# sashashura/h2o-3

Hardware: AMD Instinct MI355X
Metric: gbm_trees_per_sec (higher is better)
Workload: dtype fp32; 1 GPU; model=GBM binomial 100Mx100 ntrees=500 max_depth=8, rows=100000000, cols=100, max_depth=8, histogram_type=QuantilesGlobal, nbins=255, global_batch=100000000, parallelism=dp1

## Files before the change

### h2o3_amd/models/tree/devtree.py

```python
from __future__ import annotations

import ctypes
import os

import numpy as np
import torch

from ...ops import tree_ops
from ...ops.tree_ops import _ptr, _stream
from ...parallel import cloud
from ...parallel import collectives as coll
from ...utils import graphs
from .engine import _TreeBuf

RS = 16
(GAIN, FEAT, T, OPT, L0, L1, R0, R1, T0, T1, OK, NL, NAW, ST, CT, VAL) = range(16)
MAX_DEPTH = 11
_cv, _ci, _cll, _cd, _cf = ctypes.c_void_p, ctypes.c_int, ctypes.c_longlong, ctypes.c_double, ctypes.c_float


def _libs():
    from ...ops import _native
    lh = tree_ops._lib()
    ls = _native.get_lib("tree_split")
    if not getattr(lh, "_typed_dt", False):
        lh.h2o_dt_items.argtypes = [_ci, _cv, _ci, _ci, _ci, _ci, _ci, _cv, _cv, _cv, _cv]
        lh.h2o_dt_offsets.argtypes = [_cv, _cv, _cv, _cv, _ci, _cv, _cv, _cv, _cv]
        lh.h2o_dt_sibling.argtypes = [_cv, _cv, _cv, _ci, _ci, _ci, _ci, _ci, _ci, _cv, _cv, _cv, _cv, _cv]
        lh.h2o_dt_leaf_vals.argtypes = [_cv, _cv, _ci, _ci, _cv, _cd, _cv, _cv]
        lh.h2o_dt_root.argtypes = [_cv, _cll, _cv]
        lh.h2o_part_flags_dev.argtypes = [_cv, _ci, _cll, _cll, _cv, _cv, _cv, _ci, _cv, _cv, _ci, _cv, _cv, _cv, _cv]
        lh.h2o_part_compact_dev.argtypes = [_cv, _cv, _cv, _ci, _cv, _cv, _cv, _cv, _cv, _cv, _cv, _cv]
        lh.h2o_leaf_pos_dev.argtypes = [_cv, _cv, _ci, _ci, _cv, _cv, _cv]
        lh.h2o_leaf_scatter_dev.argtypes = [_cv, _cv, _ci, _cv, _cv, _cv, _cv]
        lh.h2o_hist_bm.argtypes = [_cv, _ci, _cv, _cv, _cv, _cv, _ci, _ci, _ci, _ci, _cf, _cf, _cv, _ci, _ci, _cv,
                                   _ci, _cll, _ci, _cv, _cv, _cv, _cv]
        lh.h2o_gbm_grad.argtypes = [_cv, _cv, _cv, _ci, _cll, _cv, _cv, _cv]
        lh.h2o_iota_i32.argtypes = [_cv, _cll, _cv]
        lh.h2o_dt_root_leaf_iota.argtypes = [_cv, _cv, _cll, _cv]
        lh.h2o_dt_colmask.argtypes = [_ci, _cv, _cv, _cv, _cv, _cv, _ci, _ci, _cv, _cv]
        lh.h2o_dt_items2.argtypes = [_ci, _cv, _ci, _ci, _ci, _ci, _ci, _cv, _cv, _cv, _cv, _cv]
        lh.h2o_leaf_flag_sums_dev.argtypes = [_cv, _cv, _cv, _ci, _cv, _cv, _ci, _ci, _cv, _cv, _cv]
        lh.h2o_leaf_gather_lds.argtypes = [_ci, _ci]
        lh.h2o_leaf_gather_items.argtypes = [_cll, _ci]
        lh.h2o_leaf_gather_dev.argtypes = [_cv, _ci, _ci, _ci, _cv, _cv, _cv, _cv, _cll, _ci, _ci, _cv, _cv, _cv, _cv,
                                           _cv, _cv]
        lh._typed_dt = True
    if not getattr(ls, "_typed_dt", False):
        ls.h2o_split_find_b.argtypes = [_cv, _ci, _ci, _ci, _cv, _cv, _cv] + [_cd] * 5 + [_ci, _cv, _cv, _ci, _cv]
        ls.h2o_split_select2.argtypes = [_cv, _cv, _ci, _ci, _ci, _ci, _cd, _ci, _cv, _cv, _cv, _cv]
        ls._typed_dt = True
    return lh, ls


def _ck(rc, what):
    if rc != 0:
        raise RuntimeError(f"{what} failed: error {rc}")


def supported(drv) -> str | None:
    if os.environ.get("H2O3_DEV_TREE", "1") != "1":
        return "disabled (H2O3_DEV_TREE=0)"
    bd, gp, p = drv.bd, drv.gp, drv.est._parms
    if drv.dev.type != "cuda":
        return "no GPU"
    if drv.K != 1 or drv.dist.family not in ("bernoulli", "gaussian") or drv.dist.link not in ("logit", "identity"):
        return "distribution"
    if drv.mono_on or drv.noise_bw != 0 or gp.interaction_sets:
        return "constraints / prediction noise"
    if not drv._base_unit:
        return "row weights other than 0/1"
    if any(bd.is_cat) or bd.code_bytes != 1 or bd.Bs > 256 or bd.Bs % 4 or bd.Fp % 16:
        return "categorical features / wide codes"
    if getattr(bd, "hist_type", "auto") in ("uniformadaptive", "random", "roundrobin"):
        return "adaptive histogram type"
    if gp.max_depth > MAX_DEPTH or gp.max_depth < 1:
        return "max_depth"
    if (gp.mtries or -1) > 0:
        return "mtries"
    if gp.max_leaves:
        return "max_leaves"
    if tree_ops.bm_groups(bd.F, bd.Fp, bd.Bs, True) is None:
        return "histogram layout"
    if drv.offset is not None or getattr(drv.dist, "huber_delta", None) is not None:
        return "offset"
    if not drv.grower.pos_payload_ok():
        return "payload path"
    return None


def gather_rows(n):
    ev = tree_ops.env("H2O3_LEAF_GATHER_R")
    return int(ev) if ev else 8192


class LeafGather:

    def __init__(self, lh, N, D, dev, R=None):
        self.lh, self.N, self.D = lh, int(N), int(D)
# ... 8 lines not shown

    def run(self, rec, ridx, vals, dbuf, flags=None, slot_wb=None):
        last = 0 if slot_wb is None else 1
        _ck(self.lh.h2o_leaf_gather_dev(_ptr(rec), self.nh, self.D, last, _ptr(slot_wb), _ptr(ridx), _ptr(flags),
                                        _ptr(vals), self.N, self.R, self.scap, _ptr(self.segs), _ptr(self.items),
                                        _ptr(self.nseg), _ptr(self.T), _ptr(dbuf), _stream()), "leaf_gather_dev")


class DevTreeGBM:

    def __init__(self, drv):
        self.drv = drv
        bd, gp = drv.bd, drv.gp
        self.bd, self.gp = bd, gp
        self.lh, self.ls = _libs()
        g = drv.grower
        self.W, self.rank = g.W, g.rank
        self.F, self.Fl, self.Fpad, self.f0 = bd.F, g.Fl, g.Fpad, g.f0
        self.N = N = bd.nrows_local
        self.D = D = int(gp.max_depth)
        self.nh = (1 << (D + 1)) - 1
        self.Bs = Bs = bd.Bs
        self.C = C = 2
        self.bern = drv.dist.family == "bernoulli"
        self.maxabs = float(drv.est._parms.get("max_abs_leafnode_pred", 1.79e308))
        dev = drv.dev
        self.dev = dev
        self.pack = tree_ops.env("H2O3_HIST_PACK", "1") == "1"
        self.ragged = tree_ops.bm_ragged()
        n_fg, G = tree_ops.bm_groups(bd.F, bd.Fp, Bs, self.pack)
        self.n_fg, self.G = n_fg, G
        self.root_ident = D >= 2 and tree_ops.env("H2O3_DEV_ROOT_IDENT", "1") != "0" and self.pack and G == 64 \
            and tree_ops.env("H2O3_HIST_BM_LW", "2") != "1"
        self.chunk_r = tree_ops.hist_chunk(N, n_fg)
        self.chunk_c = tree_ops.hist_chunk((N + 1) // 2, n_fg)
        if self.pack and max(self.chunk_r, self.chunk_c) >= (1 << 23):
            raise RuntimeError("devtree: histogram chunk too large for the packed path")
        self.chunk_p = tree_ops._part_chunk(N)
        self.chunk_l = 65536
        self.vmax = [1.0, 1.0]
        self._scales()
        n_lvl_max = 1 << (D - 1) if D >= 1 else 1
        self.cap_r = 1 + N // self.chunk_r + 1
        self.cap_c = n_lvl_max + ((N + 1) // 2) // self.chunk_c + 2
        self.cap_p = (1 << D) + N // self.chunk_p + 1
        self.cap_l = self.nh + N // self.chunk_l + 1
        cap_h = max(self.cap_r, self.cap_c)
        i32, f64 = torch.int32, torch.float64
        self.rec = torch.zeros(self.nh * RS, dtype=f64, device=dev)
        self.sums = torch.zeros(self.nh * 2, dtype=f64, device=dev)
        self.vals = torch.zeros(self.nh, dtype=torch.float32, device=dev)
        self.lr_t = torch.zeros(1, dtype=torch.float32, device=dev)
        self.ridx = [g.ridx, g.ridx2]
        self.pos = [torch.empty(N, dtype=torch.float32, device=dev) for _ in range(2)]
        self.dbuf = torch.zeros(N, dtype=torch.float32, device=dev)
        lvl = self.Fl * n_lvl_max * Bs * C
        self.Hbuf = [torch.zeros(lvl, dtype=f64, device=dev) for _ in range(2)]
        self.wyybuf = [torch.zeros(n_lvl_max, dtype=f64, device=dev) for _ in range(2)]
        npar_max = max(1, n_lvl_max // 2)
        self.Hb = torch.zeros(bd.F * npar_max * Bs * C + npar_max, dtype=f64, device=dev)
        self.Hroot = torch.zeros(bd.F * Bs * C + 1, dtype=f64, device=dev)
        self.hwork = torch.zeros(cap_h * 4, dtype=i32, device=dev)
        self.pwork = torch.zeros(self.cap_p * 4, dtype=i32, device=dev)
        self.fbase = torch.zeros(self.cap_p, dtype=i32, device=dev)
        self.lwork = torch.zeros(self.cap_l * 4, dtype=i32, device=dev)
        self.counts = torch.zeros(2, dtype=i32, device=dev)
        self.cnt = torch.zeros(self.cap_p, dtype=i32, device=dev)
        self.loff = torch.zeros(self.cap_p, dtype=i32, device=dev)
        self.roff = torch.zeros(self.cap_p, dtype=i32, device=dev)
        self.flags = torch.zeros(N // 64 + self.cap_p + 1, dtype=torch.int64, device=dev)
        self.part = tree_ops.bm_part(cap_h, n_fg, Bs, G, self.pack, dev)
        self.split_out = torch.zeros(n_lvl_max * max(self.Fl, 1) * 4, dtype=f64, device=dev)
        self.mask = torch.zeros(n_lvl_max * Bs, dtype=torch.uint8, device=dev)
        self.feat_i = torch.zeros(n_lvl_max, dtype=i32, device=dev)
        self.okm = torch.ones((n_lvl_max, max(self.Fl, 1)), dtype=torch.uint8, device=dev)
        if self.f0 + self.Fl > self.F:
            self.okm[:, max(0, self.F - self.f0):] = 0
        self._okm_col = None
        self.mono = torch.zeros(max(self.Fl, 1), dtype=torch.float32, device=dev)
        if bd.codes_col is not None:
            self.pcodes, self.prs, self.pfs = bd.codes_col, 1, bd.nrows_local
        else:
            self.pcodes, self.prs, self.pfs = bd.codes, bd.Fp, 1
        self.cutmat = g._cut_matrix()
        self.sampled = not drv._unit_weights
        self.wbuf = torch.ones(N, dtype=torch.float32, device=dev) if self.sampled else None
        self.colsamp = gp.col_sample_rate < 1.0 or gp.col_sample_rate_change_per_level != 1.0
        if self.colsamp:
            self.cs_elig = torch.zeros(max(self.F, 1), dtype=torch.int64, device=dev)
            self.cs_m = torch.zeros(1, dtype=torch.int32, device=dev)
            self.cs_k = torch.zeros(max(D, 1), dtype=torch.int32, device=dev)
            self.cs_seed = torch.zeros(max(D, 1), dtype=torch.int64, device=dev)
        self.gather = os.environ.get("H2O3_LEAF_GATHER", "1") != "0" and N > 0
        self.last_level = self.gather and os.environ.get("H2O3_DEV_LAST_LEVEL", "1") != "0"
        self.lg = LeafGather(self.lh, N, D, dev) if self.gather else None
        self.slot_wb = torch.zeros(n_lvl_max, dtype=i32, device=dev)
        self.graph = None
        self._hv = [None, None]
        self._k = 0

    def _scales(self):
        vm = self.vmax
        self.s_r = [tree_ops.fixed_point_scale(m, self.chunk_r) for m in vm]
        self.s_c = [tree_ops.fixed_point_scale(m, self.chunk_c) for m in vm]
        self.bq_r = self.bq_c = -1
        if self.pack:
            self.s_r[1], self.bq_r = tree_ops._pack_scale(vm[1], self.chunk_r)
            self.s_c[1], self.bq_c = tree_ops._pack_scale(vm[1], self.chunk_c)

    def set_tree_cols(self, mask):
        key = None if mask is None else mask.tobytes()
        if key == self._okm_col:
            return
        self._okm_col = key
        m = np.ones(self.Fpad, dtype=np.uint8)
        if mask is not None:
            m[:self.F] = np.asarray(mask, dtype=np.uint8)
        m[self.F:] = 0
        row = self._upload([m[self.f0:self.f0 + self.Fl].copy()])[0]
        self.okm.copy_(row.view(1, -1).expand_as(self.okm))

    def _upload(self, arrays):
        offs, n = [], 0
        for a in arrays:
            offs.append(n)
            n += (a.nbytes + 7) & ~7
        n = max(n, 8)
        if getattr(self, "_stg", None) is None or self._stg[0].numel() < n:
            self._stg = [torch.empty(n, dtype=torch.uint8, pin_memory=True) for _ in range(2)]
            self._stg_ev = [None, None]
            self._dstg = torch.empty(n, dtype=torch.uint8, device=self.dev)
            self._stg_i = 0
        i = self._stg_i
        self._stg_i ^= 1
        if self._stg_ev[i] is not None:
            self._stg_ev[i].synchronize()
        buf = self._stg[i].numpy()
        for a, o in zip(arrays, offs):
            buf[o:o + a.nbytes] = np.ascontiguousarray(a).view(np.uint8).reshape(-1)
        self._dstg[:n].copy_(self._stg[i][:n], non_blocking=True)
        ev = torch.cuda.Event()
        ev.record()
        self._stg_ev[i] = ev
        out = []
        for a, o in zip(arrays, offs):
            out.append(self._dstg[o:o + a.nbytes].view(torch.from_numpy(a[:0]).dtype)
                       if a.nbytes else torch.empty(0, dtype=torch.from_numpy(a[:0]).dtype, device=self.dev))
        return out

    def _rec_lvl(self, d):
        off = (1 << d) - 1
        return self.rec[off * RS:]

    def _ridx_ptr(self, d, cur):
        return None if (d == 0 and self.root_ident) else _ptr(self.ridx[cur])

    def _hist(self, d, cur):
        lh = self.lh
        bd, Bs, C = self.bd, self.Bs, self.C
        n = 1 << d
        H = self.Hbuf[d % 2][:self.Fl * n * Bs * C]
        wyy = self.wyybuf[d % 2][:n]
        s = _stream()
        if d == 0:
            _ck(lh.h2o_dt_items(0, _ptr(self.rec), 1, self.D, 0, self.chunk_r, self.cap_r, _ptr(self.hwork), None,
                                _ptr(self.counts), s), "dt_items(root)")
            nh = bd.F * Bs * C
            buf = self.Hroot
            buf.zero_()
            tree_ops.set_bm_ragged(lh, self.ragged)
            _ck(lh.h2o_hist_bm(_ptr(bd.codes), bd.Fp, self._ridx_ptr(0, cur), _ptr(self.pos[cur]), None,
                               _ptr(self.hwork), self.cap_r, bd.F, 0, Bs, self.s_r[0], self.s_r[1], _ptr(buf), 1, 0,
                               _ptr(buf[nh:]), 1, self.bq_r, self.G, None, _ptr(self.counts), _ptr(self.part), s),
                "hist_bm(root)")
            Hl, wl = buf[:nh].view(bd.F, 1, Bs, C), buf[nh:]
            if self.W > 1:
                Hl, wl = self.drv.grower._rs_hist_wyy(Hl, wl)
            H.view(self.Fl, 1, Bs, C).copy_(Hl)
            wyy.copy_(wl)
            return H, wyy
        npar = n // 2
        rp = self._rec_lvl(d - 1)
        _ck(lh.h2o_dt_items(1, _ptr(rp), npar, self.D, 0, self.chunk_c, self.cap_c, _ptr(self.hwork), None,
                            _ptr(self.counts), s), "dt_items(child)")
        nhb = bd.F * npar * Bs * C
        buf = self.Hb[:nhb + npar]
        buf.zero_()
        tree_ops.set_bm_ragged(lh, self.ragged)
        _ck(lh.h2o_hist_bm(_ptr(bd.codes), bd.Fp, _ptr(self.ridx[cur]), _ptr(self.pos[cur]), None, _ptr(self.hwork),
                           self.cap_c, bd.F, 0, Bs, self.s_c[0], self.s_c[1], _ptr(buf), npar, 0, _ptr(buf[nhb:]), 1,
                           self.bq_c, self.G, None, _ptr(self.counts), _ptr(self.part), s), "hist_bm(child)")
        Hb, wb = buf[:nhb].view(bd.F, npar, Bs, C), buf[nhb:]
        if self.W > 1:
            Hb, wb = self.drv.grower._rs_hist_wyy(Hb, wb)
            Hb, wb = Hb.contiguous(), wb.contiguous()
        Hp = self.Hbuf[(d - 1) % 2]
        wp = self.wyybuf[(d - 1) % 2]
        _ck(lh.h2o_dt_sibling(_ptr(Hb), _ptr(Hp), _ptr(rp), npar, self.Fl, Bs * C, C, 0b1, 0, _ptr(H), _ptr(wb),
                              _ptr(wp), _ptr(wyy), _stream()), "dt_sibling")
        return H, wyy

    def _merge(self, recl, n):
        W, Bs = self.W, self.Bs
        rows = recl[:n * RS].view(n, RS)
        rb = 13 * 8
        buf = torch.cat([rows[:, :13].contiguous().view(torch.uint8).view(n, rb), self.mask[:n * Bs].view(n, Bs)], 1)
        g = coll.all_gather_dim0(buf).view(W, n, rb + Bs)
        gains = g[:, :, :8].contiguous().view(torch.float64).view(W, n)
        best = torch.argmax(gains, 0)
        win = g[best, torch.arange(n, device=buf.device)]
        pk = win[:, :rb].contiguous().view(torch.float64).view(n, 13)
        rows[:, :13].copy_(pk)
        self.mask[:n * Bs].view(n, Bs).copy_(win[:, rb:])
        okf = pk[:, OK] > 0
        self.feat_i[:n].copy_(torch.where(okf, pk[:, FEAT], torch.zeros_like(pk[:, FEAT])).to(torch.int32))

    def _level(self, d, cur):
        lh, ls, gp = self.lh, self.ls, self.gp
        n = 1 << d
        Bs = self.Bs
        H, wyy = self._hist(d, cur)
        recl = self._rec_lvl(d)
        s = _stream()
        if self.colsamp:
            rp = self._rec_lvl(d - 1) if d > 0 else None
            _ck(lh.h2o_dt_colmask(d, _ptr(rp), _ptr(self.cs_elig), _ptr(self.cs_m), _ptr(self.cs_k),
                                  _ptr(self.cs_seed), self.f0, self.Fl, _ptr(self.okm), s), "dt_colmask")
        _ck(ls.h2o_split_find_b(_ptr(H), self.Fl, n, Bs, _ptr(wyy), _ptr(self.okm), _ptr(self.mono),
                                float(gp.min_rows), float(gp.min_split_improvement), float(gp.reg_lambda),
                                float(gp.reg_alpha), float(gp.gamma), 0, _ptr(self.split_out), None, 0, s),
            "split_find")
        _ck(ls.h2o_split_select2(_ptr(self.split_out), _ptr(H), self.Fl, n, Bs, self.f0, 2.0 * float(gp.min_rows), RS,
                                 _ptr(recl), _ptr(self.mask), _ptr(self.feat_i), s), "split_select2")
        if self.W > 1:
            self._merge(recl, n)
        s = _stream()
        skip = self.last_level and d == self.D - 1
        _ck(lh.h2o_dt_items2(0, _ptr(recl), n, self.D, 0, self.chunk_p, self.cap_p, _ptr(self.pwork),
                             _ptr(self.fbase), _ptr(self.slot_wb) if skip else None, _ptr(self.counts), s),
            "dt_items(part)")
        _ck(lh.h2o_part_flags_dev(_ptr(self.pcodes), 1, self.prs, self.pfs, self._ridx_ptr(d, cur),
                                  _ptr(self.pwork), _ptr(self.fbase), self.cap_p, _ptr(self.feat_i), _ptr(self.mask),
                                  Bs, _ptr(self.flags), _ptr(self.cnt), _ptr(self.counts), s), "part_flags_dev")
        _ck(lh.h2o_dt_offsets(_ptr(self.cnt), _ptr(self.pwork), _ptr(self.counts), _ptr(recl), n,
                              _ptr(self._rec_lvl(d + 1)), _ptr(self.loff), _ptr(self.roff), s), "dt_offsets")
        if skip:
            _ck(lh.h2o_leaf_flag_sums_dev(_ptr(self.pos[cur]), _ptr(self.pwork), _ptr(self.fbase), self.cap_p,
                                          _ptr(self.flags), _ptr(recl), self.D, 1 if self.bern else 0,
                                          _ptr(self.sums), _ptr(self.counts), s), "leaf_flag_sums_dev")
            return cur
        nxt = cur ^ 1
        if d == 0 and self.root_ident:
            _ck(lh.h2o_dt_root_leaf_iota(_ptr(recl), _ptr(self.ridx[0]), self.N, s), "dt_root_leaf_iota")
        _ck(lh.h2o_part_compact_dev(self._ridx_ptr(d, cur), _ptr(self.pwork), _ptr(self.fbase), self.cap_p,
                                    _ptr(self.flags), _ptr(self.loff), _ptr(self.roff), _ptr(self.ridx[nxt]),
                                    _ptr(self.pos[cur]), _ptr(self.pos[nxt]), _ptr(self.counts), s),
            "part_compact_dev")
        return nxt

    def _sequence(self):
        lh, drv = self.lh, self.drv
        s = _stream()
        y = drv.yb if self.bern else torch.nan_to_num(drv.yf)
        if not hasattr(self, "_y"):
            self._y = y.contiguous().to(torch.float32)
        f = drv._f[:, 0]
        _ck(lh.h2o_gbm_grad(_ptr(self._y), _ptr(f), _ptr(self.wbuf) if self.sampled else None,
                            1 if self.bern else 0, self.N, _ptr(self.pos[0]), _ptr(self.dbuf), s), "gbm_grad")
        if not self.root_ident:
            _ck(lh.h2o_iota_i32(_ptr(self.ridx[0]), self.N, s), "iota")
        self.rec.zero_()
        self.sums.zero_()
        _ck(lh.h2o_dt_root(_ptr(self.rec), self.N, _stream()), "dt_root")
        cur = 0
        for d in range(self.D):
            cur = self._level(d, cur)
        s = _stream()
        _ck(lh.h2o_dt_items(3 if self.last_level else 2, _ptr(self.rec), self.nh, self.D, 0, self.chunk_l, self.cap_l,
                            _ptr(self.lwork), None, _ptr(self.counts), s), "dt_items(leaf)")
        _ck(lh.h2o_leaf_pos_dev(_ptr(self.pos[cur]), _ptr(self.lwork), self.cap_l, 1 if self.bern else 0,
                                _ptr(self.sums), _ptr(self.counts), s), "leaf_pos_dev")
        if self.W > 1:
            coll.allreduce_(self.sums)
        s = _stream()
        _ck(lh.h2o_dt_leaf_vals(_ptr(self.rec), _ptr(self.sums), self.nh, self.D, _ptr(self.lr_t), self.maxabs,
                                _ptr(self.vals), s), "dt_leaf_vals")
        if self.gather:
            self.lg.run(self.rec, self.ridx[cur], self.vals, self.dbuf, self.flags if self.last_level else None,
                        self.slot_wb if self.last_level else None)
        else:
            _ck(lh.h2o_leaf_scatter_dev(_ptr(self.ridx[cur]), _ptr(self.lwork), self.cap_l, _ptr(self.vals),
                                        _ptr(self.dbuf), _ptr(self.counts), s), "leaf_scatter_dev")
        self.cur = cur

    def set_col_sampling(self, tree_mask):
        if not self.colsamp:
            return
        g, gp, F, D = self.drv.grower, self.gp, self.F, self.D
        base = np.ones(F, dtype=bool) if tree_mask is None else np.asarray(tree_mask, dtype=bool)
        elig = np.nonzero(base)[0]
        m = int(elig.size)
        ks = np.zeros(D, dtype=np.int32)
        seeds = np.zeros(D, dtype=np.int64)
        for d in range(D):
            rate = gp.col_sample_rate * (gp.col_sample_rate_change_per_level ** d)
            k = max(1, int(np.floor(rate * m + 0.5))) if rate < 1.0 else m
            if k >= m:
                ks[d] = m
            else:
                ks[d] = k
                seeds[d] = int(g.rng.randint(0, 2 ** 31 - 1))
        e = np.zeros(max(F, 1), dtype=np.int64)
        e[:m] = elig
        de, dm, dk, dsd = self._upload([e, np.array([m], dtype=np.int32), ks, seeds])
        self.cs_elig.copy_(de)
        self.cs_m.copy_(dm)
        self.cs_k.copy_(dk)
        self.cs_seed.copy_(dsd)

    def run(self, lr, pending, w=None):
        if not pending:
            self.dbuf.zero_()
        if self.sampled:
            self.wbuf.copy_(w)
        self.lr_t.fill_(float(lr))
        if not self.bern:
            f = self.drv._f[:, 0]
            z = (torch.nan_to_num(self.drv.yf) - (f + self.dbuf))
            self.vmax = [1.0, float(z.abs().max())]
# ... 73 lines not shown
```

### h2o3_amd/ops/csrc/tree_hist.hip

```cpp
#include "common.h"
#include <stdlib.h>
#include <algorithm>

template <int MODE> struct Chan { static constexpr int C = MODE == 2 ? 1 : 2; };

template <typename CodeT, int MODE, bool HAS_VB, bool POSV, bool PACK = false>
__global__ __launch_bounds__(512) void hist_build_kernel(
    const CodeT* __restrict__ codes, int Fp, const int* __restrict__ ridx,
    const float* __restrict__ va, const float* __restrict__ vb,
    const int4* __restrict__ work, int F, int Bs, int FGL, float s0, float s1,
    double* __restrict__ hist, int n_slots, double* __restrict__ wyy_out, const uint8_t* __restrict__ need,
    long long bq = 0) {
  constexpr int C = Chan<MODE>::C;
  constexpr int CL = PACK ? 1 : C;
  const int RPW = 64 / FGL;
  extern __shared__ __attribute__((aligned(16))) unsigned long long ldsq[];
  const int4 wk = work[blockIdx.x];
  if (need != nullptr && need[(size_t)wk.x * gridDim.y + blockIdx.y] == 0) return;
  const int fg0 = blockIdx.y * FGL;
  const int nf = min(FGL, F - fg0);
  const int stride_f = Bs * CL;
  const int total = FGL * stride_f;
  for (int i = threadIdx.x; i < total; i += blockDim.x) ldsq[i] = 0ull;
  __syncthreads();
// ... 821 lines not shown
  const int lane = lane_id(), wv = wave_id();
  for (int base = wk.y; base < end; base += 256 * 16) {
    const int p0 = base + threadIdx.x * 16;
    int r[16], c[16];
    unsigned bits = 0;
    int nl = 0, nv = 0;
    if (p0 < end) {
      load_items<CodeT>(codes, rs, fs, f, ridx, p0, end, r, c);
#pragma unroll
      for (int k = 0; k < 16; ++k) {
        const bool v = p0 + k < end;
        const bool L = v && m[c[k]];
        bits |= (L ? 1u : 0u) << k;
        nl += L ? 1 : 0;
        nv += v ? 1 : 0;
      }
    }
    int incl = nl;
#pragma unroll
    for (int d = 1; d < 64; d <<= 1) {
      const int u = __shfl_up(incl, d, 64);
      if (lane >= d) incl += u;
    }
    if (lane == 63) wsum[wv] = incl;
    __syncthreads();
    int wpre = 0, tot = 0;
#pragma unroll
    for (int w = 0; w < 4; ++w) {
      const int s = wsum[w];
      wpre += (w < wv) ? s : 0;
      tot += s;
    }
    const int lpre = wpre + incl - nl;
    const int tile_first = base;
    const int pos_before = max(0, min(p0, end) - tile_first);
    int li = lbase + lpre;
    int ri = rbase + (pos_before - lpre);
    if (p0 < end) {
#pragma unroll
      for (int k = 0; k < 16; ++k) {
        if (p0 + k < end) {
          const int dst = ((bits >> k) & 1u) ? li++ : ri++;
          out[dst] = r[k];
          if (pa) { pa_out[dst] = pa[p0 + k]; pb_out[dst] = pb[p0 + k]; }
        }
      }
    }
    const int tile_n = min(256 * 16, end - base);
    lbase += tot;
    rbase += tile_n - tot;
    __syncthreads();
  }
}
template <typename CodeT>
__global__ __launch_bounds__(256) void part_flags_kernel(
    const CodeT* __restrict__ codes, long long rs, long long fs, const int* __restrict__ ridx,
    const int4* __restrict__ work, const int* __restrict__ fbase, const int* __restrict__ feat,
    const uint8_t* __restrict__ masks, int Bs, unsigned long long* __restrict__ flags, int* __restrict__ cnt,
    const int* __restrict__ nw_dev) {
  __shared__ uint8_t m[4096];
  __shared__ int red[4];
  if (nw_dev != nullptr && (int)blockIdx.x >= nw_dev[1]) return;
  const int4 wk = work[blockIdx.x];
  const int f = feat[wk.x];
  for (int i = threadIdx.x; i < Bs; i += blockDim.x) m[i] = masks[(size_t)wk.x * Bs + i];
  __syncthreads();
  const int lane = threadIdx.x & 63, wv = threadIdx.x >> 6;
  const int end = wk.y + wk.z;
  const int fb = fbase[blockIdx.x];
  int local = 0;
  constexpr int U = 8;
  for (int base = wk.y; base < end; base += 256 * U) {
    int r[U], c[U];
#pragma unroll
    for (int u = 0; u < U; ++u) {
      const int pc = min(base + u * 256 + (int)threadIdx.x, end - 1);
      r[u] = ridx != nullptr ? ridx[pc] : pc;
    }
#pragma unroll
    for (int u = 0; u < U; ++u) c[u] = (int)codes[(size_t)r[u] * rs + (size_t)f * fs];
#pragma unroll
    for (int u = 0; u < U; ++u) {
      const int p = base + u * 256 + (int)threadIdx.x;
      const bool L = p < end && m[c[u]];
      const unsigned long long bal = __ballot(L);
      const int w0 = base + u * 256 + wv * 64;
      if (lane == 0 && w0 < end) flags[fb + (w0 - wk.y) / 64] = bal;
      local += L ? 1 : 0;
    }
  }
  local = (int)wave_sum((float)local);
  if (lane == 0) red[wv] = local;
  __syncthreads();
  if (threadIdx.x == 0) cnt[blockIdx.x] = red[0] + red[1] + red[2] + red[3];
}

template <int U>
__global__ __launch_bounds__(256) void part_compact_kernel(
    const int* __restrict__ ridx, const int4* __restrict__ work, const int* __restrict__ fbase,
    const unsigned long long* __restrict__ flags, const int* __restrict__ loff, const int* __restrict__ roff,
    int* __restrict__ out, const float* __restrict__ pa, float* __restrict__ pa_out, const int* __restrict__ nw_dev) {
  __shared__ int wl[U][4], wr_[U][4];
  if (nw_dev != nullptr && (int)blockIdx.x >= nw_dev[1]) return;
  const int4 wk = work[blockIdx.x];
  const int lane = threadIdx.x & 63, wv = threadIdx.x >> 6;
  const int end = wk.y + wk.z;
  const int fb = fbase[blockIdx.x];
  int lbase = loff[blockIdx.x], rbase = roff[blockIdx.x];
  const unsigned long long below = (lane == 0) ? 0ull : (~0ull >> (64 - lane));
  for (int base = wk.y; base < end; base += 256 * U) {
    int r[U];
    float a[U];
    unsigned long long bal[U], valid[U];
#pragma unroll
    for (int u = 0; u < U; ++u) {
      const int p = base + u * 256 + (int)threadIdx.x;
      const int pc = min(p, end - 1);
      r[u] = ridx != nullptr ? ridx[pc] : pc;
      a[u] = pa ? pa[pc] : 0.f;
      const int w0 = base + u * 256 + wv * 64;
      bal[u] = (w0 < end) ? flags[fb + (w0 - wk.y) / 64] : 0ull;
    }
#pragma unroll
    for (int u = 0; u < U; ++u) {
      valid[u] = __ballot(base + u * 256 + (int)threadIdx.x < end);
      const int nl_w = __popcll(bal[u] & valid[u]);
      if (lane == 0) { wl[u][wv] = nl_w; wr_[u][wv] = __popcll(valid[u]) - nl_w; }
    }
    __syncthreads();
    int lrun = 0, rrun = 0;
#pragma unroll
    for (int u = 0; u < U; ++u) {
      int lpre = lrun, rpre = rrun;
#pragma unroll
      for (int w = 0; w < 4; ++w) {
        lpre += (w < wv) ? wl[u][w] : 0;
        rpre += (w < wv) ? wr_[u][w] : 0;
// ... 1343 lines not shown

int h2o_leaf_scatter_dev(const int* ridx, const int* work, int n_cap, const float* val, float* d, const int* counts,
                         hipStream_t s) {
  if (n_cap <= 0) return 0;
  hipLaunchKernelGGL(leaf_scatter_kernel, dim3(n_cap), dim3(256), 0, s, ridx, (const int4*)work, val, d, counts);
  return (int)hipGetLastError();
}

int h2o_leaf_flag_sums_dev(const float* zp, const int* work, const int* fbase, int n_cap,
                           const unsigned long long* flags, const double* rec_lvl, int D, int mode, double* out,
                           const int* counts, hipStream_t s) {
  if (n_cap <= 0) return 0;
  if (D < 1) return -1;
  hipLaunchKernelGGL(leaf_flag_sums_kernel, dim3(n_cap), dim3(256), 0, s, zp, (const int4*)work, fbase, flags, rec_lvl,
                     (1 << (D - 1)) - 1, mode, out, counts);
  return (int)hipGetLastError();
}

#define LG_CHK 8192
int h2o_leaf_gather_lds(int R, int scap) { return (R + 2 * scap + 1) * (int)sizeof(int); }
int h2o_leaf_gather_items(long long N, int scap) { return (int)(scap + N / LG_CHK + 1); }

int h2o_leaf_gather_dev(const double* rec, int nh, int D, int last, const int* slot_wb, const int* ridx,
                        const unsigned long long* flags, const float* vals, long long N, int R, int scap, int* segs,
                        int* items, int* nseg, int* T, float* d, hipStream_t s) {
  if (N <= 0) return 0;
  if (nh <= 0 || D < 1 || R < 256 || (R & (R - 1)) != 0 || scap < (1 << D) || scap > LG_MAXSEG ||
      N > (1ll << 31) - (1 << 24))
    return -1;
  if (last != 0 && (slot_wb == nullptr || flags == nullptr)) return -1;
  const int lds = h2o_leaf_gather_lds(R, scap);
  if (lds > 160 * 1024 - 256) return -1;
  static int lds_set = 0;
  if (lds > lds_set) {
    if (hipFuncSetAttribute((const void*)lg_gather_kernel, hipFuncAttributeMaxDynamicSharedMemorySize, lds) !=
        hipSuccess)
      return -2;
    lds_set = lds;
  }
  const int nb = (int)((N + R - 1) / R);
  const int icap = h2o_leaf_gather_items(N, scap);
  const int nt = min(1024, max(256, R / 16));
  hipLaunchKernelGGL(lg_segs_kernel, dim3(1), dim3(1024), 0, s, rec, nh, D, last, slot_wb, scap, N, LG_CHK, icap,
                     (int4*)segs, (int2*)items, nseg);
  hipLaunchKernelGGL(lg_bounds_kernel, dim3(icap), dim3(256), 0, s, ridx, (const int4*)segs, nseg,
                     (const int2*)items, 31 - __builtin_clz(R), nb, scap, LG_CHK, T);
  hipLaunchKernelGGL(lg_gather_kernel, dim3(nb), dim3(nt), lds, s, ridx, (const int4*)segs, nseg, T, scap, flags,
                     vals, N, R, d);
  return (int)hipGetLastError();
}

}

extern "C" __global__ __launch_bounds__(1024) void dt_colmask_kernel(
    int d, const double* __restrict__ rec_par, const long long* __restrict__ elig, const int* __restrict__ m_dev,
    const int* __restrict__ k_dev, const unsigned long long* __restrict__ seed_dev, int f0, int Fl,
    unsigned char* __restrict__ okm) {
  __shared__ int wsum[16];
  __shared__ int carry;
  const int n = 1 << d;
  const int m = m_dev[0], k = k_dev[d];
  const unsigned long long seed = seed_dev[d];
  const int lane = threadIdx.x & 63, wv = threadIdx.x >> 6, nwv = blockDim.x >> 6;
  if (threadIdx.x == 0) carry = 0;
  __syncthreads();
  for (int base = 0; base < n; base += blockDim.x) {
    const int i = base + threadIdx.x;
    int ex = 0;
    if (i < n) ex = d == 0 ? 1 : (rec_par[(size_t)(i >> 1) * DT_RS + DT_OK] > 0.0 ? 1 : 0);
    int a = ex;
#pragma unroll
    for (int o = 1; o < 64; o <<= 1) {
      const int t = __shfl_up(a, o, 64);
      if (lane >= o) a += t;
    }
    if (lane == 63) wsum[wv] = a;
    __syncthreads();
    if (wv == 0) {
      int x = lane < nwv ? wsum[lane] : 0;
#pragma unroll
      for (int o = 1; o < 16; o <<= 1) {
        const int t = __shfl_up(x, o, 64);
        if (lane >= o) x += t;
      }
      if (lane < nwv) wsum[lane] = x;
    }
    __syncthreads();
    const int rank = carry + (wv > 0 ? wsum[wv - 1] : 0) + a - ex;
    if (i < n) {
      unsigned char* row = okm + (size_t)i * Fl;
      for (int f = 0; f < Fl; ++f) row[f] = 0;
      if (ex) {
        const unsigned long long b0 = smix64(seed ^ ((unsigned long long)rank * 0xD1B54A32D192ED03ull));
        int taken = 0;
        for (int j = 0; j < m && taken < k; ++j) {
          const double u = (double)(smix64(b0 + (unsigned long long)j) >> 11) * (1.0 / 9007199254740992.0);
          if (u * (double)(m - j) < (double)(k - taken)) {
            ++taken;
            const long long f = elig[j] - f0;
            if (f >= 0 && f < Fl) row[f] = 1;
          }
        }
      }
    }
    __syncthreads();
    if (threadIdx.x == 0) carry += wsum[nwv - 1];
// ... 14 lines not shown
```

Measured before the change: 69.49 trees/s.

## Track per-level row split decisions as bit planes instead of leaf gather

Adds a row-bits path that stores each row's left/right decision at every level as a packed bitplane in row order. Partition flags are then read from the bitplane instead of re-reading feature codes. The final leaf sums and leaf value writes are computed by streaming over rows and rebuilding each row's path from the bitplanes, which replaces the ridx-based leaf gather. This avoids random gathers and code re-reads at the cost of a full-N streaming decide pass per level, an extra pos buffer, and shared-memory atomics for the leaf sums.

```diff
diff --git a/h2o3_amd/models/tree/devtree.py b/h2o3_amd/models/tree/devtree.py
--- a/h2o3_amd/models/tree/devtree.py
+++ b/h2o3_amd/models/tree/devtree.py
@@ -16,6 +16,8 @@
 RS = 16
 (GAIN, FEAT, T, OPT, L0, L1, R0, R1, T0, T1, OK, NL, NAW, ST, CT, VAL) = range(16)
 MAX_DEPTH = 11
+ROW_BITS_DEFAULT = "1"
+ROW_BITS_THR = 128
 _cv, _ci, _cll, _cd, _cf = ctypes.c_void_p, ctypes.c_int, ctypes.c_longlong, ctypes.c_double, ctypes.c_float
 
 
@@ -45,6 +47,14 @@
         lh.h2o_leaf_gather_items.argtypes = [_cll, _ci]
         lh.h2o_leaf_gather_dev.argtypes = [_cv, _ci, _ci, _ci, _cv, _cv, _cv, _cv, _cll, _ci, _ci, _cv, _cv, _cv, _cv,
                                            _cv, _cv]
+        lh.h2o_rb_prep.argtypes = [_cv, _cv, _cv, _ci, _ci, _cv, _cv, _cv, _cv]
+        lh.h2o_rb_decide.argtypes = [_cv, _cv, _cll, _cll, _ci, _cv, _cv, _cv, _cv, _ci, _cv]
+        lh.h2o_rb_root_plane.argtypes = [_cv, _cv, _cv, _cll, _cv]
+        lh.h2o_part_flags_bits_dev.argtypes = [_cv, _cv, _cv, _cv, _ci, _cv, _cv, _cv, _cv]
+        lh.h2o_rb_leaf_sums.argtypes = [_cv, _cv, _cll, _ci, _cv, _ci, _cv, _cv, _cv]
+        lh.h2o_rb_leaf_sums_ws.argtypes = [_ci]
+        lh.h2o_rb_leaf_sums_ws.restype = _cll
+        lh.h2o_rb_leaf_rows.argtypes = [_cv, _cll, _ci, _cv, _cv, _cv, _cv]
         lh._typed_dt = True
     if not getattr(ls, "_typed_dt", False):
         ls.h2o_split_find_b.argtypes = [_cv, _ci, _ci, _ci, _cv, _cv, _cv] + [_cd] * 5 + [_ci, _cv, _cv, _ci, _cv]
@@ -159,7 +169,10 @@
         self.vals = torch.zeros(self.nh, dtype=torch.float32, device=dev)
         self.lr_t = torch.zeros(1, dtype=torch.float32, device=dev)
         self.ridx = [g.ridx, g.ridx2]
-        self.pos = [torch.empty(N, dtype=torch.float32, device=dev) for _ in range(2)]
+        self.gather = os.environ.get("H2O3_LEAF_GATHER", "1") != "0" and N > 0
+        self.last_level = self.gather and os.environ.get("H2O3_DEV_LAST_LEVEL", "1") != "0"
+        self.row_bits = self.last_level and os.environ.get("H2O3_DEV_ROW_BITS", ROW_BITS_DEFAULT) != "0"
+        self.pos = [torch.empty(N, dtype=torch.float32, device=dev) for _ in range(3 if self.row_bits else 2)]
         self.dbuf = torch.zeros(N, dtype=torch.float32, device=dev)
         lvl = self.Fl * n_lvl_max * Bs * C
         self.Hbuf = [torch.zeros(lvl, dtype=f64, device=dev) for _ in range(2)]
@@ -198,10 +211,17 @@
             self.cs_m = torch.zeros(1, dtype=torch.int32, device=dev)
             self.cs_k = torch.zeros(max(D, 1), dtype=torch.int32, device=dev)
             self.cs_seed = torch.zeros(max(D, 1), dtype=torch.int64, device=dev)
-        self.gather = os.environ.get("H2O3_LEAF_GATHER", "1") != "0" and N > 0
-        self.last_level = self.gather and os.environ.get("H2O3_DEV_LAST_LEVEL", "1") != "0"
-        self.lg = LeafGather(self.lh, N, D, dev) if self.gather else None
+        self.lg = LeafGather(self.lh, N, D, dev) if self.gather and not self.row_bits else None
         self.slot_wb = torch.zeros(n_lvl_max, dtype=i32, device=dev)
+        if self.row_bits:
+            self.nw = -(-N // 64)
+            self.rowbits = torch.zeros(D * self.nw, dtype=torch.int64, device=dev)
+            self.rb_ft = torch.zeros(n_lvl_max, dtype=i32, device=dev)
+            self.rb_mk = torch.zeros(n_lvl_max * 8, dtype=i32, device=dev)
+            self.rb_nd = torch.zeros(1, dtype=i32, device=dev)
+            self.rb_part = torch.zeros(self.lh.h2o_rb_leaf_sums_ws(D), dtype=f64, device=dev)
+            ev = tree_ops.env("H2O3_ROW_BITS_THR")
+            self.rb_thr = int(ev) if ev else ROW_BITS_THR
         self.graph = None
         self._hv = [None, None]
         self._k = 0
@@ -259,6 +279,11 @@
         off = (1 << d) - 1
         return self.rec[off * RS:]
 
+    def _pos(self, d, cur):
+        if self.row_bits:
+            return self.pos[0 if d == 0 else 1 + ((d - 1) & 1)]
+        return self.pos[cur]
+
     def _ridx_ptr(self, d, cur):
         return None if (d == 0 and self.root_ident) else _ptr(self.ridx[cur])
 
@@ -276,7 +301,7 @@
             buf = self.Hroot
             buf.zero_()
             tree_ops.set_bm_ragged(lh, self.ragged)
-            _ck(lh.h2o_hist_bm(_ptr(bd.codes), bd.Fp, self._ridx_ptr(0, cur), _ptr(self.pos[cur]), None,
+            _ck(lh.h2o_hist_bm(_ptr(bd.codes), bd.Fp, self._ridx_ptr(0, cur), _ptr(self._pos(0, cur)), None,
                                _ptr(self.hwork), self.cap_r, bd.F, 0, Bs, self.s_r[0], self.s_r[1], _ptr(buf), 1, 0,
                                _ptr(buf[nh:]), 1, self.bq_r, self.G, None, _ptr(self.counts), _ptr(self.part), s),
                 "hist_bm(root)")
@@ -294,7 +319,7 @@
         buf = self.Hb[:nhb + npar]
         buf.zero_()
         tree_ops.set_bm_ragged(lh, self.ragged)
-        _ck(lh.h2o_hist_bm(_ptr(bd.codes), bd.Fp, _ptr(self.ridx[cur]), _ptr(self.pos[cur]), None, _ptr(self.hwork),
+        _ck(lh.h2o_hist_bm(_ptr(bd.codes), bd.Fp, _ptr(self.ridx[cur]), _ptr(self._pos(d, cur)), None, _ptr(self.hwork),
                            self.cap_c, bd.F, 0, Bs, self.s_c[0], self.s_c[1], _ptr(buf), npar, 0, _ptr(buf[nhb:]), 1,
                            self.bq_c, self.G, None, _ptr(self.counts), _ptr(self.part), s), "hist_bm(child)")
         Hb, wb = buf[:nhb].view(bd.F, npar, Bs, C), buf[nhb:]
@@ -341,6 +366,8 @@
                                  _ptr(recl), _ptr(self.mask), _ptr(self.feat_i), s), "split_select2")
         if self.W > 1:
             self._merge(recl, n)
+        if self.row_bits:
+            return self._level_rb(d, cur, recl, n)
         s = _stream()
         skip = self.last_level and d == self.D - 1
         _ck(lh.h2o_dt_items2(0, _ptr(recl), n, self.D, 0, self.chunk_p, self.cap_p, _ptr(self.pwork),
@@ -365,6 +392,55 @@
             "part_compact_dev")
         return nxt
 
+    def _level_rb(self, d, cur, recl, n):
+        lh, bd, s = self.lh, self.bd, _stream()
+        if d == 0 and self.D > 1:
+            _ck(lh.h2o_dt_items2(0, _ptr(recl), n, self.D, 0, self.chunk_p, self.cap_p, _ptr(self.pwork),
+                                 _ptr(self.fbase), None, _ptr(self.counts), s), "dt_items(part)")
+            _ck(lh.h2o_part_flags_dev(_ptr(self.pcodes), 1, self.prs, self.pfs, self._ridx_ptr(d, cur),
+                                      _ptr(self.pwork), _ptr(self.fbase), self.cap_p, _ptr(self.feat_i),
+                                      _ptr(self.mask), self.Bs, _ptr(self.flags), _ptr(self.cnt), _ptr(self.counts),
+                                      s), "part_flags_dev")
+            _ck(lh.h2o_rb_root_plane(_ptr(self.flags), _ptr(recl), _ptr(self.rowbits), self.N, s), "rb_root_plane")
+            return self._compact_rb(d, cur, recl, n)
+        _ck(lh.h2o_rb_prep(_ptr(self.feat_i), _ptr(self.mask), _ptr(recl), n, self.Bs, _ptr(self.rb_ft),
+                           _ptr(self.rb_mk), _ptr(self.rb_nd), s), "rb_prep")
+        _ck(lh.h2o_rb_decide(_ptr(bd.codes_col) if bd.codes_col is not None else None, _ptr(bd.codes), bd.Fp, self.N,
+                             d, _ptr(self.rb_ft), _ptr(self.rb_mk), _ptr(self.rowbits), _ptr(self.rb_nd), self.rb_thr,
+                             s), "rb_decide")
+        if d == self.D - 1:
+            return cur
+        _ck(lh.h2o_dt_items2(0, _ptr(recl), n, self.D, 0, self.chunk_p, self.cap_p, _ptr(self.pwork),
+                             _ptr(self.fbase), None, _ptr(self.counts), s), "dt_items(part)")
+        _ck(lh.h2o_part_flags_bits_dev(_ptr(self.rowbits[d * self.nw:]), self._ridx_ptr(d, cur), _ptr(self.pwork),
+                                       _ptr(self.fbase), self.cap_p, _ptr(self.flags), _ptr(self.cnt),
+                                       _ptr(self.counts), s), "part_flags_bits_dev")
+        return self._compact_rb(d, cur, recl, n)
+
+    def _compact_rb(self, d, cur, recl, n):
+        lh, s = self.lh, _stream()
+        _ck(lh.h2o_dt_offsets(_ptr(self.cnt), _ptr(self.pwork), _ptr(self.counts), _ptr(recl), n,
+                              _ptr(self._rec_lvl(d + 1)), _ptr(self.loff), _ptr(self.roff), s), "dt_offsets")
+        nxt = cur ^ 1
+        _ck(lh.h2o_part_compact_dev(self._ridx_ptr(d, cur), _ptr(self.pwork), _ptr(self.fbase), self.cap_p,
+                                    _ptr(self.flags), _ptr(self.loff), _ptr(self.roff), _ptr(self.ridx[nxt]),
+                                    _ptr(self._pos(d, cur)), _ptr(self._pos(d + 1, nxt)), _ptr(self.counts), s),
+            "part_compact_dev")
+        return nxt
+
+    def _tail_rb(self):
+        lh = self.lh
+        _ck(lh.h2o_rb_leaf_sums(_ptr(self.pos[0]), _ptr(self.rowbits), self.N, self.D, _ptr(self.rec),
+                                1 if self.bern else 0, _ptr(self.rb_part), _ptr(self.sums), _stream()),
+            "rb_leaf_sums")
+        if self.W > 1:
+            coll.allreduce_(self.sums)
+        s = _stream()
+        _ck(lh.h2o_dt_leaf_vals(_ptr(self.rec), _ptr(self.sums), self.nh, self.D, _ptr(self.lr_t), self.maxabs,
+                                _ptr(self.vals), s), "dt_leaf_vals")
+        _ck(lh.h2o_rb_leaf_rows(_ptr(self.rowbits), self.N, self.D, _ptr(self.rec), _ptr(self.vals), _ptr(self.dbuf),
+                                s), "rb_leaf_rows")
+
     def _sequence(self):
         lh, drv = self.lh, self.drv
         s = _stream()
@@ -382,6 +458,9 @@
         cur = 0
         for d in range(self.D):
             cur = self._level(d, cur)
+        self.cur = cur
+        if self.row_bits:
+            return self._tail_rb()
         s = _stream()
         _ck(lh.h2o_dt_items(3 if self.last_level else 2, _ptr(self.rec), self.nh, self.D, 0, self.chunk_l, self.cap_l,
                             _ptr(self.lwork), None, _ptr(self.counts), s), "dt_items(leaf)")
diff --git a/h2o3_amd/ops/csrc/tree_hist.hip b/h2o3_amd/ops/csrc/tree_hist.hip
--- a/h2o3_amd/ops/csrc/tree_hist.hip
+++ b/h2o3_amd/ops/csrc/tree_hist.hip
@@ -897,19 +897,22 @@
     __syncthreads();
   }
 }
-template <typename CodeT>
+template <typename CodeT, bool BITS = false>
 __global__ __launch_bounds__(256) void part_flags_kernel(
     const CodeT* __restrict__ codes, long long rs, long long fs, const int* __restrict__ ridx,
     const int4* __restrict__ work, const int* __restrict__ fbase, const int* __restrict__ feat,
     const uint8_t* __restrict__ masks, int Bs, unsigned long long* __restrict__ flags, int* __restrict__ cnt,
-    const int* __restrict__ nw_dev) {
-  __shared__ uint8_t m[4096];
+    const int* __restrict__ nw_dev, const unsigned int* __restrict__ plane = nullptr) {
+  __shared__ uint8_t m[BITS ? 4 : 4096];
   __shared__ int red[4];
   if (nw_dev != nullptr && (int)blockIdx.x >= nw_dev[1]) return;
   const int4 wk = work[blockIdx.x];
-  const int f = feat[wk.x];
-  for (int i = threadIdx.x; i < Bs; i += blockDim.x) m[i] = masks[(size_t)wk.x * Bs + i];
-  __syncthreads();
+  int f = 0;
+  if constexpr (!BITS) {
+    f = feat[wk.x];
+    for (int i = threadIdx.x; i < Bs; i += blockDim.x) m[i] = masks[(size_t)wk.x * Bs + i];
+    __syncthreads();
+  }
   const int lane = threadIdx.x & 63, wv = threadIdx.x >> 6;
   const int end = wk.y + wk.z;
   const int fb = fbase[blockIdx.x];
@@ -923,11 +926,16 @@
       r[u] = ridx != nullptr ? ridx[pc] : pc;
     }
 #pragma unroll
-    for (int u = 0; u < U; ++u) c[u] = (int)codes[(size_t)r[u] * rs + (size_t)f * fs];
+    for (int u = 0; u < U; ++u) {
+      if constexpr (BITS) c[u] = (int)((plane[r[u] >> 5] >> (r[u] & 31)) & 1u);
+      else c[u] = (int)codes[(size_t)r[u] * rs + (size_t)f * fs];
+    }
 #pragma unroll
     for (int u = 0; u < U; ++u) {
       const int p = base + u * 256 + (int)threadIdx.x;
-      const bool L = p < end && m[c[u]];
+      bool L;
+      if constexpr (BITS) L = p < end && c[u] != 0;
+      else L = p < end && m[c[u]];
       const unsigned long long bal = __ballot(L);
       const int w0 = base + u * 256 + wv * 64;
       if (lane == 0 && w0 < end) flags[fb + (w0 - wk.y) / 64] = bal;
@@ -2377,6 +2385,309 @@
 
 }
 
+#define RB_MW 8
+#define RB_MAXD 11
+#define RB_FBITS 65536
+
+__global__ __launch_bounds__(256) void rb_prep_kernel(const int* __restrict__ feat, const uint8_t* __restrict__ masks,
+                                                      const double* __restrict__ rec_lvl, int n, int Bs,
+                                                      int* __restrict__ ft, unsigned int* __restrict__ mk,
+                                                      int* __restrict__ ndist) {
+  const int it = blockIdx.x * 256 + threadIdx.x;
+  if (it < n * RB_MW) {
+    const int i = it / RB_MW, w = it % RB_MW;
+    const bool ok = rec_lvl[(size_t)i * DT_RS + DT_OK] > 0.0;
+    unsigned int bits = 0;
+    if (ok)
+      for (int b = 0; b < 32; ++b) {
+        const int c = w * 32 + b;
+        if (c < Bs && masks[(size_t)i * Bs + c]) bits |= 1u << b;
+      }
+    mk[it] = bits;
+    if (w == 0) ft[i] = ok ? feat[i] : -1;
+  }
+  if (blockIdx.x != 0) return;
+  __shared__ unsigned int bm[RB_FBITS / 32];
+  __shared__ int tot;
+  for (int k = threadIdx.x; k < RB_FBITS / 32; k += 256) bm[k] = 0;
+  if (threadIdx.x == 0) tot = 0;
+  __syncthreads();
+  for (int i = threadIdx.x; i < n; i += 256)
+    if (rec_lvl[(size_t)i * DT_RS + DT_OK] > 0.0) {
+      const int f = feat[i];
+      if (f >= 0 && f < RB_FBITS) atomicOr(&bm[f >> 5], 1u << (f & 31));
+      else atomicAdd(&tot, 1);
+    }
+  __syncthreads();
+  int c = 0;
+  for (int k = threadIdx.x; k < RB_FBITS / 32; k += 256) c += __popc(bm[k]);
+  if (c) atomicAdd(&tot, c);
+  __syncthreads();
+  if (threadIdx.x == 0) ndist[0] = tot;
+}
+
+#define RB_U 8
+template <int DL>
+__global__ __launch_bounds__(256) void rb_decide_kernel(
+    const uint8_t* __restrict__ col, const uint8_t* __restrict__ rm, long long Fp, long long N,
+    const int* __restrict__ ft_g, const unsigned int* __restrict__ mk_g,
+    const unsigned long long* __restrict__ above, unsigned long long* __restrict__ out, long long NW,
+    const int* __restrict__ ndist, int thr) {
+  extern __shared__ unsigned int rb_lds[];
+  constexpr int n = 1 << DL;
+  int* ft = (int*)rb_lds;
+  unsigned int* mk = rb_lds + n;
+  for (int i = threadIdx.x; i < n; i += 256) ft[i] = ft_g[i];
+  for (int i = threadIdx.x; i < n * RB_MW; i += 256) mk[i] = mk_g[i];
+  __syncthreads();
+  const bool use_col = col != nullptr && ndist[0] <= thr;
+  const uint8_t* __restrict__ cb = use_col ? col : rm;
+  const size_t rs = use_col ? (size_t)1 : (size_t)Fp, fs = use_col ? (size_t)N : (size_t)1;
+  const int lane = threadIdx.x & 63;
+  const long long nwave = (long long)gridDim.x * 4;
+  for (long long w0 = ((long long)blockIdx.x * 4 + (threadIdx.x >> 6)) * RB_U; w0 < NW; w0 += nwave * RB_U) {
+    const long long wu = (long long)__builtin_amdgcn_readfirstlane((int)w0);
+    int slot[RB_U];
+#pragma unroll
+    for (int u = 0; u < RB_U; ++u) slot[u] = 0;
+#pragma unroll
+    for (int l = 0; l < DL; ++l) {
+#pragma unroll
+      for (int u = 0; u < RB_U; ++u) {
+        const unsigned long long wd = above[(long long)l * NW + min(wu + u, NW - 1)];
+        slot[u] = 2 * slot[u] + (int)(((wd >> lane) & 1ull) ^ 1ull);
+      }
+    }
+    int f[RB_U], c[RB_U];
+#pragma unroll
+    for (int u = 0; u < RB_U; ++u) {
+      const long long r = (wu + u) * 64 + lane;
+      f[u] = r < N ? ft[slot[u]] : -1;
+      c[u] = (int)cb[(size_t)min(r, N - 1) * rs + (size_t)max(f[u], 0) * fs];
+    }
+#pragma unroll
+    for (int u = 0; u < RB_U; ++u) {
+      const bool L = f[u] >= 0 && ((mk[slot[u] * RB_MW + (c[u] >> 5)] >> (c[u] & 31)) & 1u);
+      const unsigned long long bal = __ballot(L);
+      if (lane == 0 && wu + u < NW) out[wu + u] = bal;
+    }
+  }
+}
+
+__device__ __forceinline__ void rb_ok_bits(const double* __restrict__ rec, int D, unsigned int* okb) {
+  for (int k = threadIdx.x; k < (1 << RB_MAXD) / 32; k += blockDim.x) okb[k] = 0;
+  __syncthreads();
+  for (int h = threadIdx.x; h < (1 << D) - 1; h += blockDim.x)
+    if (rec[(size_t)h * DT_RS + DT_OK] > 0.0) atomicOr(&okb[h >> 5], 1u << (h & 31));
+  __syncthreads();
+}
+__device__ __forceinline__ int rb_leaf_of_path(const unsigned int* okb, int p, int D) {
+  int h = 0;
+  for (int l = 0; l < D; ++l) {
+    if (!((okb[h >> 5] >> (h & 31)) & 1u)) break;
+    h = 2 * h + 1 + ((p >> (D - 1 - l)) & 1);
+  }
+  return h;
+}
+template <int D>
+__device__ __forceinline__ void rb_paths8(const unsigned long long* __restrict__ rowbits, long long NW, long long q,
+                                          int path[8]) {
+  const uint8_t* pb = (const uint8_t*)rowbits;
+  unsigned int b[D];
+#pragma unroll
+  for (int l = 0; l < D; ++l) b[l] = pb[(size_t)l * (size_t)NW * 8 + (size_t)q];
+#pragma unroll
+  for (int k = 0; k < 8; ++k) path[k] = 0;
+#pragma unroll
+  for (int l = 0; l < D; ++l) {
+#pragma unroll
+    for (int k = 0; k < 8; ++k) path[k] = 2 * path[k] + (int)(((b[l] >> k) & 1u) ^ 1u);
+  }
+}
+
+__global__ __launch_bounds__(256) void rb_root_plane_kernel(const unsigned long long* __restrict__ flags,
+                                                            const double* __restrict__ rec,
+                                                            unsigned long long* __restrict__ plane, long long NW) {
+  const bool ok = rec[DT_OK] > 0.0;
+  for (long long w = (long long)blockIdx.x * 256 + threadIdx.x; w < NW; w += (long long)gridDim.x * 256)
+    plane[w] = ok ? flags[w] : 0ull;
+}
+
+template <int D>
+__global__ __launch_bounds__(256) void rb_leaf_sums_kernel(const float* __restrict__ z,
+                                                           const unsigned long long* __restrict__ rowbits,
+                                                           long long NW, long long N,
+                                                           int mode, int ncopy, double* __restrict__ part) {
+  extern __shared__ double rb_acc[];
+  const int np = 1 << D;
+  for (int i = threadIdx.x; i < ncopy * np * 2; i += blockDim.x) rb_acc[i] = 0.0;
+  __syncthreads();
+  double* acc = rb_acc + (size_t)(threadIdx.x >> 6) * np * 2;
+  const long long nq = (N + 7) >> 3;
+  for (long long q = (long long)blockIdx.x * blockDim.x + threadIdx.x; q < nq;
+       q += (long long)gridDim.x * blockDim.x) {
+    float zz[8];
+    if (8 * q + 7 < N) {
+      const float4 v = *(const float4*)(z + 8 * q), w = *(const float4*)(z + 8 * q + 4);
+      zz[0] = v.x; zz[1] = v.y; zz[2] = v.z; zz[3] = v.w;
+      zz[4] = w.x; zz[5] = w.y; zz[6] = w.z; zz[7] = w.w;
+    } else {
+#pragma unroll
+      for (int k = 0; k < 8; ++k) zz[k] = 8 * q + k < N ? z[8 * q + k] : __builtin_nanf("");
+    }
+    int path[8];
+    rb_paths8<D>(rowbits, NW, q, path);
+#pragma unroll
+    for (int k = 0; k < 8; ++k) {
+      if (zz[k] == zz[k]) {
+        const double az = fabs((double)zz[k]);
+        const double b = mode == 1 ? az * (1.0 - az) : 1.0;
+        __hip_atomic_fetch_add(&acc[2 * path[k]], (double)zz[k], __ATOMIC_RELAXED, __HIP_MEMORY_SCOPE_WORKGROUP);
+        __hip_atomic_fetch_add(&acc[2 * path[k] + 1], b, __ATOMIC_RELAXED, __HIP_MEMORY_SCOPE_WORKGROUP);
+      }
+    }
+  }
+  __syncthreads();
+  for (int i = threadIdx.x; i < np * 2; i += blockDim.x) {
+    double v = 0.0;
+    for (int k = 0; k < ncopy; ++k) v += rb_acc[(size_t)k * np * 2 + i];
+    part[(size_t)blockIdx.x * np * 2 + i] = v;
+  }
+}
+
+__global__ __launch_bounds__(256) void rb_leaf_sums_reduce_kernel(const double* __restrict__ part, int nb, int D,
+                                                                  const double* __restrict__ rec,
+                                                                  double* __restrict__ sums) {
+  const int np2 = 2 << D;
+  const int i = blockIdx.x * 4 + (threadIdx.x >> 6), lane = threadIdx.x & 63;
+  if (i >= np2) return;
+  double v = 0.0;
+  for (int b = lane; b < nb; b += 64) v += part[(size_t)b * np2 + i];
+  v = wave_sum(v);
+  if (lane == 0 && v != 0.0) {
+    const int p = i >> 1;
+    int h = 0;
+    for (int l = 0; l < D; ++l) {
+      if (!(rec[(size_t)h * DT_RS + DT_OK] > 0.0)) break;
+      h = 2 * h + 1 + ((p >> (D - 1 - l)) & 1);
+    }
+    gbl_add(sums + 2 * (size_t)h + (i & 1), v);
+  }
+}
+
+template <int D>
+__global__ __launch_bounds__(256) void rb_leaf_rows_kernel(const unsigned long long* __restrict__ rowbits,
+                                                           long long NW, long long N,
+                                                           const double* __restrict__ rec,
+                                                           const float* __restrict__ vals, float* __restrict__ dout) {
+  __shared__ float tv[1 << RB_MAXD];
+  __shared__ unsigned int okb[(1 << RB_MAXD) / 32];
+  rb_ok_bits(rec, D, okb);
+  for (int p = threadIdx.x; p < (1 << D); p += 256) tv[p] = vals[rb_leaf_of_path(okb, p, D)];
+  __syncthreads();
+  const long long nq = (N + 7) >> 3;
+  for (long long q = (long long)blockIdx.x * 256 + threadIdx.x; q < nq; q += (long long)gridDim.x * 256) {
+    int path[8];
+    rb_paths8<D>(rowbits, NW, q, path);
+    if (8 * q + 7 < N) {
+      *(float4*)(dout + 8 * q) = make_float4(tv[path[0]], tv[path[1]], tv[path[2]], tv[path[3]]);
+      *(float4*)(dout + 8 * q + 4) = make_float4(tv[path[4]], tv[path[5]], tv[path[6]], tv[path[7]]);
+    } else {
+#pragma unroll
+      for (int k = 0; k < 8; ++k)
+        if (8 * q + k < N) dout[8 * q + k] = tv[path[k]];
+    }
+  }
+}
+
+extern "C" {
+
+int h2o_rb_prep(const int* feat, const uint8_t* masks, const double* rec_lvl, int n, int Bs, int* ft,
+                unsigned int* mk, int* ndist, hipStream_t s) {
+  if (n <= 0 || n > (1 << (RB_MAXD - 1)) || Bs <= 0 || Bs > RB_MW * 32) return -1;
+  hipLaunchKernelGGL(rb_prep_kernel, dim3((n * RB_MW + 255) / 256), dim3(256), 0, s, feat, masks, rec_lvl, n, Bs, ft,
+                     mk, ndist);
+  return (int)hipGetLastError();
+}
+
+#define RB_BY_D(D, X)                                                                                           \
+  switch (D) {                                                                                                  \
+    case 0: X(0); break; case 1: X(1); break; case 2: X(2); break; case 3: X(3); break;                         \
+    case 4: X(4); break; case 5: X(5); break; case 6: X(6); break; case 7: X(7); break;                         \
+    case 8: X(8); break; case 9: X(9); break; case 10: X(10); break; default: X(11); break;                     \
+  }
+
+int h2o_rb_decide(const uint8_t* col, const uint8_t* rm, long long Fp, long long N, int d, const int* ft,
+                  const unsigned int* mk, unsigned long long* rowbits, const int* ndist, int thr, hipStream_t s) {
+  if (N <= 0) return 0;
+  if (d < 0 || d > RB_MAXD - 1 || rm == nullptr || N > (1ll << 31) - (1 << 24)) return -1;
+  const long long NW = (N + 63) / 64;
+  const long long nb = (NW + 4 * RB_U - 1) / (4 * RB_U);
+  const size_t lds = (size_t)(1 << d) * (1 + RB_MW) * sizeof(unsigned int);
+  const dim3 grid((unsigned)std::min<long long>(nb, 4096));
+#define RB_K1(DD)                                                                                                  \
+  hipLaunchKernelGGL(rb_decide_kernel<(DD < 11 ? DD : 10)>, grid, dim3(256), lds, s, col, rm, Fp, N, ft, mk,       \
+                     (const unsigned long long*)rowbits, rowbits + (size_t)d * NW, NW, ndist, thr)
+  RB_BY_D(d, RB_K1)
+#undef RB_K1
+  return (int)hipGetLastError();
+}
+
+int h2o_rb_root_plane(const unsigned long long* flags, const double* rec, unsigned long long* rowbits, long long N,
+                      hipStream_t s) {
+  if (N <= 0) return 0;
+  const long long NW = (N + 63) / 64;
+  hipLaunchKernelGGL(rb_root_plane_kernel, dim3((unsigned)std::min<long long>((NW + 255) / 256, 2048)), dim3(256), 0,
+                     s, flags, rec, rowbits, NW);
+  return (int)hipGetLastError();
+}
+
+int h2o_part_flags_bits_dev(const unsigned long long* plane, const int* ridx, const int* work, const int* fbase,
+                            int n_cap, unsigned long long* flags, int* cnt, const int* counts, hipStream_t s) {
+  if (n_cap <= 0) return 0;
+  hipLaunchKernelGGL((part_flags_kernel<uint8_t, true>), dim3(n_cap), dim3(256), 0, s, (const uint8_t*)nullptr, 0ll,
+                     0ll, ridx, (const int4*)work, fbase, (const int*)nullptr, (const uint8_t*)nullptr, 0, flags, cnt,
+                     counts, (const unsigned int*)plane);
+  return (int)hipGetLastError();
+}
+
+static int rb_leaf_copies(int D) { return std::max(1, std::min(4, (32 * 1024) / ((1 << D) * 16))); }
+#define RB_LS_BLOCKS 2048
+long long h2o_rb_leaf_sums_ws(int D) { return (long long)RB_LS_BLOCKS * (2ll << D); }
+
+int h2o_rb_leaf_sums(const float* z, const unsigned long long* rowbits, long long N, int D, const double* rec,
+                     int mode, double* part, double* sums, hipStream_t s) {
+  if (N <= 0) return 0;
+  if (D < 1 || D > RB_MAXD || part == nullptr) return -1;
+  const long long NW = (N + 63) / 64, nq = (N + 7) / 8;
+  const int ncopy = rb_leaf_copies(D), nt = 64 * ncopy;
+  const size_t lds = (size_t)ncopy * (1 << D) * 2 * sizeof(double);
+  const int nb = (int)std::min<long long>((nq + nt - 1) / nt, RB_LS_BLOCKS);
+#define RB_LS(DD)                                                                                                  \
+  hipLaunchKernelGGL(rb_leaf_sums_kernel<(DD > 0 ? DD : 1)>, dim3(nb), dim3(nt), lds, s, z, rowbits, NW, N, mode,  \
+                     ncopy, part)
+  RB_BY_D(D, RB_LS)
+#undef RB_LS
+  hipLaunchKernelGGL(rb_leaf_sums_reduce_kernel, dim3(((2 << D) + 3) / 4), dim3(256), 0, s, (const double*)part, nb,
+                     D, rec, sums);
+  return (int)hipGetLastError();
+}
+
+int h2o_rb_leaf_rows(const unsigned long long* rowbits, long long N, int D, const double* rec, const float* vals,
+                     float* d, hipStream_t s) {
+  if (N <= 0) return 0;
+  if (D < 1 || D > RB_MAXD) return -1;
+  const long long NW = (N + 63) / 64, nq = (N + 7) / 8;
+  const dim3 grid((unsigned)std::min<long long>((nq + 255) / 256, 2048));
+#define RB_LR(DD)                                                                                              \
+  hipLaunchKernelGGL(rb_leaf_rows_kernel<(DD > 0 ? DD : 1)>, grid, dim3(256), 0, s, rowbits, NW, N, rec, vals, d)
+  RB_BY_D(D, RB_LR)
+#undef RB_LR
+  return (int)hipGetLastError();
+}
+
+}
+
 extern "C" __global__ __launch_bounds__(1024) void dt_colmask_kernel(
     int d, const double* __restrict__ rec_par, const long long* __restrict__ elig, const int* __restrict__ m_dev,
     const int* __restrict__ k_dev, const unsigned long long* __restrict__ seed_dev, int f0, int Fl,
```

Result: no change. 70.12 trees/s, median of 4 (+0.9%).
